# zhouyifan233/light-transport

Measured on AMD Instinct MI355X. Metric: photon_steps_per_sec, higher is better.
Workload: dtype f64

## Files before the change

### light_transport_amd/csrc/lt_api.cpp

```cpp
#include <hip/hip_runtime_api.h>

#include <dlfcn.h>

#include <algorithm>
#include <cmath>
#include <cctype>
#include <cstdarg>
#include <cstdio>
#include <cstdlib>
#include <cstring>
#include <limits>
#include <mutex>
#include <new>
#include <string>
#include <vector>

#include "lt_internal.hpp"

using namespace ltk;

static const size_t kMeshLdsBudget = 64 * 1024;

namespace {

// ... 635 lines not shown
    static WalkGate gates[16];
    return gates[device & 15];
}

hipError_t lane_event(LogLane& ln, hipStream_t s)
{
    if (ln.ev_used == ln.evs.size()) {
        hipEvent_t ev;
        hipError_t e = hipEventCreate(&ev);
        if (e != hipSuccess) return e;
        ln.evs.push_back(ev);
    }
    return hipEventRecord(ln.evs[ln.ev_used++], s);
}

int run_log_plan(LogRun& R, const LogPlan& plan, uint64_t offset, int* n_batches)
{
    lt_ctx* c = R.c;
    const LogGeom& G = R.G;
    const bool hot = G.bits2 != 0 && c->dmap_valid;
    const uint32_t n_hist = G.bits2 ? G.nb1 : G.n_tiles;
    LaunchCfg cfg = R.cfg;
    cfg.lds_bytes = walk_lds_bytes(R.v, R.P.n_media, R.P.n_layers, R.P.n_tris, R.P.n_nodes, n_hist);
    const int resident = walk_max_blocks_per_cu(R.v, cfg.threads, cfg.lds_bytes);
    if (resident <= 0) return c->fail(LT_E_HIP, "lt_launch: log-mode kernel not resident");
    int per_cu = c->blocks_per_cu > 0 ? c->blocks_per_cu : (plan.lanes >= 2 ? (resident + 1) / 2 : resident);
    if (plan.lanes >= 2 && c->knob.overlap_walk_bpc >= 1 && c->knob.overlap_walk_bpc <= 8) per_cu = (int)c->knob.overlap_walk_bpc;
    const unsigned long long cap = (unsigned long long)per_cu * (unsigned long long)c->prop.multiProcessorCount;
    if (plan.lanes >= 2) {
        const size_t gb = c->n_vox() * c->grid_elem();
        HIP_TRY(c, hipEventRecord(c->ev_fork, c->stream));
        for (int l = 1; l < plan.lanes; l++) {
            if (!c->lanes[l].stream) HIP_TRY(c, hipStreamCreateWithFlags(&c->lanes[l].stream, hipStreamNonBlocking));
            HIP_TRY(c, hipStreamWaitEvent(c->lanes[l].stream, c->ev_fork, 0));
            HIP_TRY(c, hipMemsetAsync(c->d_gridx[l - 1].p, 0, gb, c->lanes[l].stream));
        }
    }
    for (const auto& bt : plan.batches) {
        LogLane& ln = c->lanes[bt.first];
        hipStream_t s = ln.stream;
        uint32_t* meta = (uint32_t*)ln.meta.p;
        WalkParams P = R.P;
        P.n_photons = bt.second; P.photon_offset = offset;
        if (bt.first >= 1) P.grid = c->d_gridx[bt.first - 1].p;
        P.head = (unsigned long long*)ln.head.p;
        P.log_idx = (uint32_t*)ln.log_idx.p; P.log_val = ln.log_val.p; P.log_fill = (uint32_t*)ln.log_fill.p;
        P.log_next = meta + LM_NEXT; P.log_overflow = meta + LM_OVERFLOW; P.log_cap_chunks = plan.cap_chunks[bt.first];
// ... 14 lines not shown
        L.items2 = (uint32_t*)ln.items2.p; L.items_c = (uint32_t*)ln.items_c.p; L.items_r = (uint32_t*)ln.items_r.p;
        L.itab = (uint32_t*)ln.itab.p;
        L.meta = meta; L.job = (unsigned long long*)c->d_job.p; L.cap_chunks = P.log_cap_chunks;
        L.n_tiles = G.n_tiles; L.bits2 = G.bits2;
        L.grid = bt.first >= 1 ? c->d_gridx[bt.first - 1].p : c->d_grid.p; L.n_vox = c->n_vox(); L.tally = c->tally;
        L.nx = (uint32_t)c->nx; L.ny = (uint32_t)c->ny; L.nz = (uint32_t)c->nz; L.ntx = G.ntx; L.nty = G.nty;
        L.flush_atomic = 0;
        if (hot) { L.dmap = (const uint16_t*)c->d_dmap.p; L.dmeta = (const uint32_t*)c->d_dmeta.p; }

        HIP_TRY(c, hipMemsetAsync(ln.head.p, 0, sizeof(unsigned long long), s));
        HIP_TRY(c, hipMemsetAsync(meta, 0, LM_WORDS * 4, s));
        HIP_TRY(c, hipMemsetAsync(ln.hist.p, 0, (size_t)G.n_tiles * (G.bits2 ? kLogGroups2 : kLogGroups) * 4, s));
        HIP_TRY(c, hipMemsetAsync(ln.log_fill.p, 0, (size_t)P.log_cap_chunks * 4, s));
        if (G.bits2) HIP_TRY(c, hipMemsetAsync(ln.hist1.p, 0, (size_t)(hot ? log_max_digits() : G.nb1) * kLogGroups * 4, s));
        const bool last_batch = &bt == &plan.batches.back();
        const uint64_t waves_launched = (uint64_t)cfg.blocks * (uint64_t)(cfg.threads / 64);
        const bool big_enough = c->knob.tail_split >= 2 || bt.second >= kTailSplitMinPerWave * waves_launched;
        const bool split = R.v.mesh <= 1 && !R.v.table && !R.v.capture && c->knob.tail_split != 0 && big_enough &&
                           ((plan.lanes == 1 && (c->blocks_per_cu == 0 || c->knob.serial_walks > 0) && (!R.v.f32 || c->knob.tail_split >= 2)) ||
                            (plan.lanes > 1 && last_batch));
        L.alone = (plan.lanes == 1 && c->blocks_per_cu == 0 && !split) ? 1 : 0;
        if (c->knob.part_alone == 0 || c->knob.part_alone == 1) L.alone = (int)c->knob.part_alone;
        L.lds_part = c->knob.part_lds > 0 ? (int)(c->knob.part_lds & 7) : 0;
        Variant vw = R.v;
        if (split) {
            const size_t cap = (size_t)cfg.blocks * (size_t)(cfg.threads / 64) * kDumpPoolLanes;
            P.dump_max = c->knob.tail_split > 1 ? (uint32_t)std::min<long>(c->knob.tail_split, (long)kDumpPoolLanes) : kDumpMaxLanes;
            HIP_TRY(c, ln.pool.ensure(cap * (R.v.f32 ? sizeof(SurvD<float>) : sizeof(SurvD<double>))));
            HIP_TRY(c, ln.pool_n.ensure(4));
            if (!ln.tail_stream) HIP_TRY(c, hipStreamCreateWithFlags(&ln.tail_stream, hipStreamNonBlocking));
            if (!ln.ev_bulk) HIP_TRY(c, hipEventCreateWithFlags(&ln.ev_bulk, hipEventDisableTiming));
            if (!ln.ev_tail) HIP_TRY(c, hipEventCreateWithFlags(&ln.ev_tail, hipEventDisableTiming));
            HIP_TRY(c, hipMemsetAsync(ln.pool_n.p, 0, 4, s));
            P.pool = ln.pool.p; P.pool_n = (uint32_t*)ln.pool_n.p; P.pool_cap = (uint32_t)cap;
            vw.phase = 1;
        }
        const bool train = c->knob.serial_walks > 0;
        if (train) {
            WalkGate& g = walk_gate(c->device);
            std::lock_guard<std::mutex> lk(g.mu);
            if (g.last) HIP_TRY(c, hipStreamWaitEvent(s, g.last, 0));
        }
        HIP_TRY(c, lane_event(ln, s));
        HIP_TRY(c, launch_walk(P, vw, cfg, s));
        HIP_TRY(c, lane_event(ln, s));
        if (split) {
            HIP_TRY(c, hipEventRecord(ln.ev_bulk, s));
// ... 297 lines not shown
              uint64_t table_steps, uint32_t flags)
{
    CHECK_CTX(c);
    if (c->media.empty()) return c->fail(LT_E_STATE, "lt_launch: lt_set_media first");
    if (!c->have_layers && !c->have_mesh) return c->fail(LT_E_STATE, "lt_launch: lt_set_layers or lt_set_mesh first");
    if (!c->have_grid) return c->fail(LT_E_STATE, "lt_launch: lt_set_grid first");
    if (!c->have_source) return c->fail(LT_E_STATE, "lt_launch: lt_set_source first");
    const int n_media = (int)c->media.size();
    if (c->have_layers) {
        for (int32_t m : c->layer_medium) if (m >= n_media) return c->fail(LT_E_INVALID, "lt_launch: layer medium index %d >= %d media", m, n_media);
    } else {
        for (size_t i = 0; i < c->med_front.size(); i++)
            if (c->med_front[i] >= n_media || c->med_back[i] >= n_media || c->med_front[i] < -1 || c->med_back[i] < -1)
                return c->fail(LT_E_INVALID, "lt_launch: triangle %zu medium index out of range", i);
        if (c->start_medium < 0 || c->start_medium >= n_media) return c->fail(LT_E_INVALID, "lt_launch: start_medium out of range");
    }
    Variant v;
    v.f32 = (flags & LT_FLAG_F32_WALK) ? 1 : 0;
    v.mesh = c->have_mesh ? 1 : 0;
    v.table = rng_table ? 1 : 0;
    v.tally = c->tally;
    v.capture = c->max_vertices > 0 ? 1 : 0;
    v.phase = 0;
    if (v.capture && (v.f32 || v.table)) return c->fail(LT_E_UNSUPPORTED, "lt_launch: vertex capture runs the f64 walk with the XORWOW generator");
    if (c->on(c->knob.diag_no_tally)) v.tally = 3;
    if (v.table && v.f32) return c->fail(LT_E_UNSUPPORTED, "lt_launch: table RNG runs the f64 walk only");
    if (v.table && v.tally == LT_TALLY_F32) return c->fail(LT_E_UNSUPPORTED, "lt_launch: table RNG needs an f64 or u64fx tally");
    if (v.table && table_steps == 0) return c->fail(LT_E_INVALID, "lt_launch: table_steps == 0");
    BIND(c);
    int rc = upload_tables(c);
    if (rc) return rc;
    if (n_photons == 0) { c->timed = false; return LT_OK; }

    if (v.table) {
        const size_t bytes = (size_t)n_photons * (size_t)table_steps * 4 * sizeof(double);
        HIP_TRY(c, c->d_table.ensure(bytes));
        HIP_TRY(c, hipMemcpyAsync(c->d_table.p, rng_table, bytes, hipMemcpyHostToDevice, c->stream));
        HIP_TRY(c, hipStreamSynchronize(c->stream));
    }

    WalkParams P;
    std::memset(&P, 0, sizeof P);
    P.head = (unsigned long long*)c->d_head.p;
    P.n_photons = n_photons; P.photon_offset = photon_offset; P.seed = seed;
    const int pi = v.f32 ? 1 : 0;
    P.media = c->d_media[pi].p; P.zb = c->d_zb[pi].p; P.ifaces = c->d_if[pi].p; P.layer_medium = (const int32_t*)c->d_lm.p;
// ... 612 lines not shown
```

### light_transport_amd/csrc/lt_internal.hpp

```cpp
#pragma once
#include <hip/hip_runtime_api.h>
#include <stdint.h>

#include "../../include/lt.h"

namespace ltk {

template <typename R>
struct MedD {
    R mu_t, inv_mu_t, absorb, g;
    R n, one_m_g2, one_p_g2, inv_2g;
    R dep;
    R one_m_g, two_g;
    R pad_;
};

template <typename R>
struct IfD {
    R n_up, n_dn;
    R nr_down, nr_up;
};

template <typename R>
struct TriD {
// ... 85 lines not shown
    double corg[3], cinv[3];
    MarchGrid mg;
    void* pool;
    uint32_t* pool_n;
    uint32_t pool_cap;
    uint32_t dump_max;
    lt_vertex* vertices;
    uint32_t* vertex_counts;
    unsigned max_vertices;
};

struct LaunchCfg {
    int blocks, threads;
    size_t lds_bytes;
};

struct Variant {
    int f32;
    int mesh;
    int table;
    int tally;
    int capture;
    int phase;
};

hipError_t launch_walk(const WalkParams& P, const Variant& v, const LaunchCfg& cfg, hipStream_t s);
size_t walk_lds_bytes(const Variant& v, int n_media, int n_layers, int n_tris, int n_nodes, unsigned n_hist = 0);
int walk_max_blocks_per_cu(const Variant& v, int threads, size_t lds_bytes);

struct RenderParams {
    const void* tris;
    const void* nodes;
    const lt_surface_material* mats;
    const lt_point_light* lights;
    const int16_t* links;
    int n_tris, n_nodes, n_lights;
    int W, H, S, D;
    double cam[3], f_distance;
    const double* xs;
    const double* ys;
    double* rand_0;
    const double* rand_1;
    const int32_t* light_choice;
    double* image;
    int variant;
    int choices;
// ... 72 lines not shown
```

### light_transport_amd/csrc/lt_kernels.hip

```cpp
#include <hip/hip_runtime.h>

#define ROCRAND_DETAIL_BM_NOT_IN_STATE
#include <rocrand/rocrand_xorwow.h>
#include <rocrand/rocrand_uniform.h>

#include "lt_internal.hpp"

static_assert(sizeof(rocrand_state_xorwow) == 6 * sizeof(uint32_t), "rocrand_state_xorwow is not {d, x[5]}: SurvD::rng and the tail-split hand-over assume it");

namespace ltk {

#define LT_DEV __device__ __forceinline__
#define LT_PV(name, k) (sizeof(R) == 8 ? (R)P.name[k] : (R)P.f32.name[k])
#define LT_GV(name, k) (sizeof(R) == 8 ? (R)G.name[k] : (R)G.name##32[k])

#ifdef LT_K_IN_SGPR
LT_DEV double fma_k(double a, double b, double k) { double r; asm("v_fma_f64 %0, %1, %2, %3" : "=v"(r) : "v"(a), "v"(b), "s"(k)); return r; }
LT_DEV double fma_mk(double a, double k, double c) { return __builtin_fma(a, k, c); }
LT_DEV double mul_k(double a, double k) { return a * k; }
LT_DEV double fma_kk(double x, double k) { double r; asm("v_fma_f64 %0, %1, %2, %2" : "=v"(r) : "v"(x), "s"(k)); return r; }
#else
template <unsigned long long BITS> LT_DEV double fma_kb(double a, double b)
{
    double r;
// ... 731 lines not shown
        if (qn > 0 && (full || qn >= 64u || !__any(marching))) march_drain(tris, G, W, qn);
    }
    if (want) march_result(tris, nodes, n_nodes, (const int16_t*)nullptr, W, outside || heavy, px, py, pz, ux, uy, uz, tmax, prim, t_out);
    else { prim = -1; t_out = Mx<R>::inf(); }
}

template <typename R> LT_DEV R hg_pdf(R cos_t, R g)
{
    R denom = (R)1 + g * g + (R)2 * g * cos_t;
    return (R)0.07957747154594767 * ((R)1 - g * g) / (denom * Mx<R>::sqrt(denom));
}

template <typename R> LT_DEV R hg_sample(R xi, R g, R one_m_g2, R one_p_g2, R inv_2g)
{
    R c;
    if (g == 0) c = (R)2 * xi - (R)1;
    else {
        R t = Mx<R>::quot(one_m_g2, (R)1 - g + (R)2 * g * xi);
        c = (one_p_g2 - t * t) * inv_2g;
    }
    return Mx<R>::clamp_unit(c);
}

template <typename R> LT_DEV R hg_sample_walk(R xi, const MedD<R>* M)
{
    if (M->g == 0) return (R)2 * xi - (R)1;
    const R t = Mx<R>::quot(M->one_m_g2, M->two_g * xi + M->one_m_g);
    return (M->one_p_g2 - t * t) * M->inv_2g;
}

template <typename R> LT_DEV void onb(const R* n, R* v2, R* v3)
{
    if (Mx<R>::abs(n[0]) > Mx<R>::abs(n[1])) {
        R l = Mx<R>::sqrt(n[0] * n[0] + n[2] * n[2]);
        v2[0] = -n[2] / l; v2[1] = 0; v2[2] = n[0] / l;
    } else {
        R l = Mx<R>::sqrt(n[1] * n[1] + n[2] * n[2]);
        v2[0] = 0; v2[1] = n[2] / l; v2[2] = -n[1] / l;
    }
    cross3(n, v2, v3);
}

template <typename R, bool LEAN = false> LT_DEV void disk(R u0, R u1, R* d)
{
    R ox = (R)2 * u0 - (R)1, oy = (R)2 * u1 - (R)1;
    if (ox == 0 && oy == 0) { d[0] = 0; d[1] = 0; return; }
    R r, theta;
    if (Mx<R>::abs(ox) > Mx<R>::abs(oy)) { r = ox; theta = (R)0.7853981633974483 * (oy / ox); }
// ... 172 lines not shown
};

LT_DEV void lds_copy(void* dst, const void* src, size_t bytes)
{
    uint32_t* d = reinterpret_cast<uint32_t*>(dst);
    const uint32_t* s = reinterpret_cast<const uint32_t*>(src);
    for (size_t i = threadIdx.x; i < bytes / 4; i += blockDim.x) d[i] = s[i];
}

LT_DEV unsigned long long readlane64(unsigned long long v, int lane)
{
    unsigned lo = __builtin_amdgcn_readlane((unsigned)v, lane);
    unsigned hi = __builtin_amdgcn_readlane((unsigned)(v >> 32), lane);
    return ((unsigned long long)hi << 32) | lo;
}

template <typename T> LT_DEV T wave_sum(T v)
{
#pragma unroll
    for (int off = 32; off > 0; off >>= 1) v += __shfl_down(v, off, 64);
    return v;
}

template <typename R>
LT_DEV void record_vertex(const WalkParams& P, unsigned long long rel, unsigned& nv, R px, R py, R pz, R ux, R uy,
                          R uz, R w, int kind, int medium, unsigned step, R gx, R gy, R gz, R pdf_pos, R pdf_dir)
{
    if (nv < P.max_vertices) {
        lt_vertex* v = P.vertices + rel * (unsigned long long)P.max_vertices + nv;
        v->point[0] = (double)px; v->point[1] = (double)py; v->point[2] = (double)pz;
        v->direction[0] = (double)ux; v->direction[1] = (double)uy; v->direction[2] = (double)uz;
        v->g_norm[0] = (double)gx; v->g_norm[1] = (double)gy; v->g_norm[2] = (double)gz;
        v->throughput = (double)w; v->pdf_pos = (double)pdf_pos; v->pdf_dir = (double)pdf_dir;
        v->kind = kind; v->medium = medium; v->step = step; v->pad_ = 0;
        nv++;
        P.vertex_counts[rel] = nv;
    }
}

constexpr unsigned kLogExhausted = 0xfffffffeu;
template <int TALLY>
LT_DEV void emit_deposit(const WalkParams& P, bool has, unsigned idx, typename TallyT<TALLY>::type val,
                         unsigned& lg_cur, unsigned& lg_end, unsigned& lg_chunk, uint32_t* s_hist)
{
    typedef typename TallyT<TALLY>::type TV;
    if (P.log_idx == nullptr) {
        if (has) tally_add<TALLY>(P.grid, idx, val);
        return;
    }
    const unsigned long long m = __ballot(has);
    if (m == 0ull) return;
    const unsigned cnt = (unsigned)__popcll(m);
    if (lg_chunk != kLogExhausted && lg_end - lg_cur < cnt) {
        const int lane = threadIdx.x & 63;
        const unsigned grp = blockIdx.x & (kLogGroups - 1);
        if (lg_chunk < kLogExhausted && lane == 0) P.log_fill[lg_chunk] = lg_cur - lg_chunk * kLogChunk;
        unsigned c = 0;
        if (lane == 0) c = __hip_atomic_fetch_add(P.log_next + grp, 1u, __ATOMIC_RELAXED, __HIP_MEMORY_SCOPE_AGENT);
        c = grp + kLogGroups * __builtin_amdgcn_readfirstlane(c);
        if (c < P.log_cap_chunks) { lg_chunk = c; lg_cur = c * kLogChunk; lg_end = lg_cur + kLogChunk; }
        else { lg_chunk = kLogExhausted; lg_cur = lg_end = 0; }
    }
    if (lg_chunk == kLogExhausted) {
        if ((threadIdx.x & 63) == 0) __hip_atomic_fetch_add(P.log_overflow, cnt, __ATOMIC_RELAXED, __HIP_MEMORY_SCOPE_AGENT);
        if (has) {
            unsigned ntx = P.log_ntx, nty = P.log_nty;
            asm volatile("" : "+s"(ntx), "+s"(nty));
            const unsigned tile = idx >> kTileShift, tx = tile % ntx, ty = (tile / ntx) % nty,
                           tz = tile / (ntx * nty);
            const unsigned vx = (tx << kTileBX) | (idx & 31u), vy = (ty << kTileBY) | ((idx >> 5) & 31u),
                           vz = (tz << kTileBZ) | ((idx >> 10) & 15u);
            tally_add<TALLY>(P.grid, (vz * (unsigned)P.ny + vy) * (unsigned)P.nx + vx, val);
        }
        return;
    }
    if (has) {
        const unsigned rank = __builtin_amdgcn_mbcnt_hi((unsigned)(m >> 32), __builtin_amdgcn_mbcnt_lo((unsigned)m, 0u));
        P.log_idx[lg_cur + rank] = idx;
        reinterpret_cast<TV*>(P.log_val)[lg_cur + rank] = val;
        atomicAdd(&s_hist[idx >> P.log_hist_shift], 1u);
    }
    lg_cur += cnt;
}

constexpr unsigned kPacket = 64;
#ifndef LT_REFILL_MIN
#define LT_REFILL_MIN 4
#endif
constexpr unsigned kRefillMin = LT_REFILL_MIN;
#ifndef LT_QUERY_MIN
#define LT_QUERY_MIN 8
#endif
constexpr unsigned kQueryMin = LT_QUERY_MIN;
constexpr unsigned kQueryMinGlobal = 48;
#ifndef LT_QUERY_MAX_AGE
#define LT_QUERY_MAX_AGE 8
#endif
// ... 28 lines not shown
#define LT_WALK_NAME walk_kernel
#define LT_WALK_BATCH 0
#include "lt_walk_kernel.inc"
#undef LT_WALK_NAME
#undef LT_WALK_BATCH
#undef LT_INV_MODE
#define LT_INV_MODE LT_INV_MODE_MESH
#define LT_WALK_NAME walk_kernel_q
#define LT_WALK_BATCH 1
#include "lt_walk_kernel.inc"
#undef LT_WALK_NAME
#undef LT_WALK_BATCH
#undef LT_INV_MODE
#define LT_INV_MODE LT_INV_MODE_MARCH
#define LT_WALK_NAME walk_kernel_m
#define LT_WALK_BATCH 2
#include "lt_walk_kernel.inc"
#undef LT_WALK_NAME
#undef LT_WALK_BATCH
#undef LT_INV_MODE

typedef void (*WalkFn)(const WalkParams);

template <typename R, int GEOM, bool TABLE, bool CAPTURE>
static WalkFn pick_tally(int tally)
{
    switch (tally) {
    case LT_TALLY_F32:
        if constexpr (TABLE) return nullptr;
        else if constexpr (GEOM == 0) return walk_kernel<R, GEOM, TABLE, LT_TALLY_F32, CAPTURE>;
        else return walk_kernel_q<R, GEOM, TABLE, LT_TALLY_F32, CAPTURE>;
    case LT_TALLY_F64:
        if constexpr (GEOM == 0) return walk_kernel<R, GEOM, TABLE, LT_TALLY_F64, CAPTURE>;
        else return walk_kernel_q<R, GEOM, TABLE, LT_TALLY_F64, CAPTURE>;
    case LT_TALLY_U64FX:
        if constexpr (GEOM == 0) return walk_kernel<R, GEOM, TABLE, LT_TALLY_U64FX, CAPTURE>;
        else return walk_kernel_q<R, GEOM, TABLE, LT_TALLY_U64FX, CAPTURE>;
    case LT_TALLY_NONE:
        if constexpr (!TABLE && GEOM == 0 && !CAPTURE) return walk_kernel<R, GEOM, TABLE, LT_TALLY_NONE, false>; else return nullptr;
    }
    return nullptr;
}

template <typename R, bool CAPTURE>
static WalkFn pick_march(int tally)
{
    switch (tally) {
    case LT_TALLY_F32: return walk_kernel_m<R, 2, false, LT_TALLY_F32, CAPTURE>;
    case LT_TALLY_F64: return walk_kernel_m<R, 2, false, LT_TALLY_F64, CAPTURE>;
    case LT_TALLY_U64FX: return walk_kernel_m<R, 2, false, LT_TALLY_U64FX, CAPTURE>;
    }
    return nullptr;
}

template <typename R, bool TABLE, bool CAPTURE>
static WalkFn pick_geom(const Variant& v)
{
    if (v.mesh == 3) { if constexpr (!TABLE) return pick_march<R, CAPTURE>(v.tally); else return nullptr; }
    if (v.mesh == 0) return pick_tally<R, 0, TABLE, CAPTURE>(v.tally);
    if (v.mesh == 1) return pick_tally<R, 1, TABLE, CAPTURE>(v.tally);
    if constexpr (!TABLE) return pick_tally<R, 2, TABLE, CAPTURE>(v.tally); else return nullptr;
}

template <typename R, int PHASE>
static WalkFn pick_phase(int tally)
{
    switch (tally) {
    case LT_TALLY_F32: return walk_kernel<R, 0, false, LT_TALLY_F32, false, PHASE>;
    case LT_TALLY_F64: return walk_kernel<R, 0, false, LT_TALLY_F64, false, PHASE>;
    case LT_TALLY_U64FX: return walk_kernel<R, 0, false, LT_TALLY_U64FX, false, PHASE>;
    }
    return nullptr;
}

template <typename R, int PHASE>
static WalkFn pick_phase_q(int tally)
{
    switch (tally) {
    case LT_TALLY_F32: return walk_kernel_q<R, 1, false, LT_TALLY_F32, false, PHASE>;
    case LT_TALLY_F64: return walk_kernel_q<R, 1, false, LT_TALLY_F64, false, PHASE>;
    case LT_TALLY_U64FX: return walk_kernel_q<R, 1, false, LT_TALLY_U64FX, false, PHASE>;
    }
    return nullptr;
}

static WalkFn pick(const Variant& v)
{
    if (v.phase) {
        if (v.mesh > 1 || v.table || v.capture) return nullptr;
        if (v.mesh == 1) {
            if (v.phase == 1) return v.f32 ? pick_phase_q<float, 1>(v.tally) : pick_phase_q<double, 1>(v.tally);
            return v.f32 ? pick_phase_q<float, 2>(v.tally) : pick_phase_q<double, 2>(v.tally);
        }
        if (v.phase == 1) return v.f32 ? pick_phase<float, 1>(v.tally) : pick_phase<double, 1>(v.tally);
        return v.f32 ? pick_phase<float, 2>(v.tally) : pick_phase<double, 2>(v.tally);
    }
    if (v.capture) return (v.f32 || v.table) ? nullptr : pick_geom<double, false, true>(v);
    if (v.f32) return v.table ? nullptr : pick_geom<float, false, false>(v);
    return v.table ? pick_geom<double, true, false>(v) : pick_geom<double, false, false>(v);
}

size_t walk_lds_bytes(const Variant& v, int n_media, int n_layers, int n_tris, int n_nodes, unsigned n_hist)
{
    if (v.mesh) n_layers = 0;
    if (v.mesh != 1) { n_tris = 0; n_nodes = 0; }
    return v.f32 ? LdsLayout<float>(n_media, n_layers, n_tris, n_nodes, n_hist, v.mesh == 3 ? 4 * sizeof(MarchWave<float>) : 0).total
                 : LdsLayout<double>(n_media, n_layers, n_tris, n_nodes, n_hist, v.mesh == 3 ? 4 * sizeof(MarchWave<double>) : 0).total;
}

int walk_max_blocks_per_cu(const Variant& v, int threads, size_t lds_bytes)
{
    WalkFn fn = pick(v);
    if (!fn) return 0;
    int nb = 0;
    if (hipOccupancyMaxActiveBlocksPerMultiprocessor(&nb, reinterpret_cast<const void*>(fn), threads, lds_bytes) != hipSuccess)
        return 0;
    return nb;
}

hipError_t launch_walk(const WalkParams& Pin, const Variant& v, const LaunchCfg& cfg, hipStream_t s)
{
    WalkFn fn = pick(v);
    if (!fn) return hipErrorInvalidValue;
    WalkParams P = Pin;
    if (v.mesh) P.n_layers = 0; else { P.n_tris = 0; P.n_nodes = 0; }
    if (cfg.lds_bytes > 64 * 1024) {
        hipError_t e = hipFuncSetAttribute(reinterpret_cast<const void*>(fn),
                                           hipFuncAttributeMaxDynamicSharedMemorySize, (int)cfg.lds_bytes);
        if (e != hipSuccess) return e;
    }
    hipLaunchKernelGGL(fn, dim3(cfg.blocks), dim3(cfg.threads), cfg.lds_bytes, s, P);
    return hipGetLastError();
}

__global__ void k_intersect_rays(const TriD<double>* tris, const NodeD<double>* nodes, int n_tris, int n_nodes,
                                 const double* o, const double* d, const double* tmax, size_t n, int use_bvh,
                                 const MarchGrid G, const int16_t* links, int32_t* prim, double* t)
{
    size_t i = (size_t)blockIdx.x * blockDim.x + threadIdx.x;
    if (use_bvh == 2) {
        __shared__ MarchWave<double> mw[4];
        const bool want = i < n;
        const size_t k = want ? i : 0;
        int pi; double tt;
        march_service<double>(tris, nodes, n_nodes, G, &mw[threadIdx.x >> 6], want, o[3 * k], o[3 * k + 1], o[3 * k + 2], d[3 * k], d[3 * k + 1],
                              d[3 * k + 2], tmax ? tmax[k] : __builtin_huge_val(), 0.0, pi, tt);
// ... 698 lines not shown
```

### light_transport_amd/csrc/lt_walk_kernel.inc

```
#ifndef LT_MED
#define LT_MED(i) reinterpret_cast<const MedD<R>*>(reinterpret_cast<const unsigned char*>(s_med) + __umul24((unsigned)(i), (unsigned)sizeof(MedD<R>)))
#endif
#if LT_WALK_BATCH != 2
template <typename R, int GEOM, bool TABLE, int TALLY, bool CAPTURE, int PHASE = 0>
#else
template <typename R, int GEOM, bool TABLE, int TALLY, bool CAPTURE>
#endif
#if LT_WALK_BATCH == 0 && defined(LT_SLAB_VGPR_CAP)
__attribute__((amdgpu_num_vgpr(LT_SLAB_VGPR_CAP)))
#endif
__global__ void __launch_bounds__(256, (sizeof(R) == 8 ? (GEOM == 0 ? LT_F64_SLAB_WAVES : (GEOM == 2 ? LT_F64_GLOBAL_WAVES : LT_F64_WAVES)) : (GEOM == 0 ? LT_F32_WAVES : 4))) LT_WALK_NAME(const WalkParams P)
{
    constexpr bool MESH = GEOM != 0;
#if LT_WALK_BATCH == 2
    constexpr int PHASE = 0;
#endif
#if LT_WALK_PRIO
    __builtin_amdgcn_s_setprio(LT_WALK_PRIO);
#endif
    extern __shared__ __attribute__((aligned(16))) unsigned char lds_raw[];
    const LdsLayout<R> L(P.n_media, P.n_layers, GEOM == 1 ? P.n_tris : 0, GEOM == 1 ? P.n_nodes : 0,
                         P.log_idx ? P.log_n_hist : 0u, LT_WALK_BATCH == 2 ? 4 * sizeof(MarchWave<R>) : 0);
    uint32_t* s_hist = reinterpret_cast<uint32_t*>(lds_raw + L.off_hist);
    if (P.log_idx) for (unsigned t = threadIdx.x; t < P.log_n_hist; t += blockDim.x) s_hist[t] = 0;
    double* s_cnt = reinterpret_cast<double*>(lds_raw + L.off_cnt);
    const MedD<R>* s_med = reinterpret_cast<const MedD<R>*>(lds_raw + L.off_media);
    const R* s_zb = reinterpret_cast<const R*>(lds_raw + L.off_zb);
    const int32_t* s_lm = reinterpret_cast<const int32_t*>(lds_raw + L.off_lm);
    const IfD<R>* s_if = reinterpret_cast<const IfD<R>*>(lds_raw + L.off_if);
    const TriD<R>* s_tris = GEOM == 2 ? reinterpret_cast<const TriD<R>*>(P.tris)
                                      : reinterpret_cast<const TriD<R>*>(lds_raw + L.off_tris);
    const NodeD<R>* s_nodes = GEOM == 2 ? reinterpret_cast<const NodeD<R>*>(P.nodes)
                                        : reinterpret_cast<const NodeD<R>*>(lds_raw + L.off_nodes);

    const int16_t* s_links = !MESH || !P.links ? nullptr
                             : (GEOM == 1 ? reinterpret_cast<const int16_t*>(lds_raw + L.off_links) : P.links);
    if (threadIdx.x < 8) s_cnt[threadIdx.x] = 0.0;
    R* s_frame = reinterpret_cast<R*>(lds_raw + L.off_frame);
// ... 203 lines not shown
                    P.vertex_counts[id] = 0;
                    if (alive) {
                        R pdf_pos = 1;
                        if (P.src_type == LT_SRC_COSINE_QUAD) {
                            const R e1[3] = {(R)P.src_e1[0], (R)P.src_e1[1], (R)P.src_e1[2]}, e2[3] = {(R)P.src_e2[0], (R)P.src_e2[1], (R)P.src_e2[2]};
                            R cr[3]; cross3(e1, e2, cr);
                            pdf_pos = (R)1 / Mx<R>::sqrt(dot3(cr, cr));
                        }
                        record_vertex<R>(P, id, nv, px, py, pz, ux, uy, uz, w, LT_VERTEX_LIGHT, cur, 0u, (R)P.src_dir[0], (R)P.src_dir[1],
                                         (R)P.src_dir[2], pdf_pos, e_pdf_dir);
                    }
                }
                if constexpr (TABLE) {
                    unsigned long long cap = P.table_steps > grp ? P.table_steps - grp : 0ull;
                    if (cap < (unsigned long long)max_steps) max_steps = (unsigned)cap;
                }
            }
        }
        if constexpr (PHASE == 1) {
            if (q_done && pk_next >= pk_end && !dumped) {
                const unsigned long long am = __ballot(alive);
                const unsigned na = (unsigned)__popcll(am);
                if (na != 0u && na <= P.dump_max) {
                    emit_deposit<TALLY>(P, pend_idx != kNoVoxel, pend_idx, pend_val, lg_cur, lg_end, lg_chunk, s_hist);
                    pend_idx = kNoVoxel;
                    const int leader = __ffsll((long long)am) - 1;
                    unsigned base = 0;
                    if (lane == leader) base = __hip_atomic_fetch_add(P.pool_n, na, __ATOMIC_RELAXED, __HIP_MEMORY_SCOPE_AGENT);
                    base = (unsigned)__builtin_amdgcn_readlane((int)base, leader);
                    if (alive) {
                        const unsigned slot = base + __builtin_amdgcn_mbcnt_hi((unsigned)(am >> 32), __builtin_amdgcn_mbcnt_lo((unsigned)am, 0u));
                        if (slot < P.pool_cap) {
                            SurvD<R>& S = reinterpret_cast<SurvD<R>*>(P.pool)[slot];
                            S.p[0] = px; S.p[1] = py; S.p[2] = pz; S.u[0] = ux; S.u[1] = uy; S.u[2] = uz; S.w = w; S.sleft = sleft;
                            S.pid = 0ull; S.cur = cur; S.step = step;
                            __builtin_memcpy(S.rng, &rng, sizeof S.rng);
#if LT_WALK_BATCH == 1
                            if constexpr (!TABLE) {
                                S.q_pend = q_pend ? 1u : 0u;
                                S.held[0] = __builtin_bit_cast(uint32_t, q_u1); S.held[1] = __builtin_bit_cast(uint32_t, q_u2);
                                S.held[2] = __builtin_bit_cast(uint32_t, q_u3);
                                q_pend = false;
                            }
#else
                            S.q_pend = 0u;
#endif
                            alive = false;
// ... 214 lines not shown
#endif
            }
        }
#if defined(LT_DIAG_MESH)
        {
            const unsigned long long gm = __ballot(go), bm = __ballot(go && hit_tri >= 0);
            dg_go += __popcll(gm);
            if (bm) { dg_bnd_it++; dg_bnd += __popcll(bm); }
            if (gm & ~bm) { dg_int_it++; dg_int += __popcll(gm & ~bm); }
        }
#endif
#if defined(LT_DIAG_MESH)
        const long long dg_t1 = clock64();
#endif
        if (go) {
            {
                const MedD<R>* Mp = LT_MED(MESH ? cur : s_lm[cur]);
                const R mu_t = Mp->mu_t;
#else
        unsigned f_idx = kNoVoxel;
        TV f_val = 0;
        if (alive) {
            if (step >= max_steps) {
                atomicAdd(&s_cnt[CW_CAPPED], (double)w); alive = false;
            } else {
                step++;
                acc_steps++;
                float clr = -1.0f;
                if constexpr (GEOM == 2) {
                    if (P.mg.cell) clr = march_clearance<R>(P.mg, px, py, pz);
                } else if constexpr (MESH) {
                    if (P.clear) {
                        const R cx = (px - LT_PV(corg, 0)) * LT_PV(cinv, 0), cy = (py - LT_PV(corg, 1)) * LT_PV(cinv, 1),
                                cz = (pz - LT_PV(corg, 2)) * LT_PV(cinv, 2);
                        if (cx >= 0 && cx < LT_PV(cdim, 0) && cy >= 0 && cy < LT_PV(cdim, 1) && cz >= 0 && cz < LT_PV(cdim, 2))
                            clr = __uint_as_float(P.clear[((size_t)(int)cz * P.cny + (int)cy) * P.cnx + (int)cx].x);
                    }
                }
                R u1;
                typename HeldU<R, TABLE>::type x0, x2, x3;
                if constexpr (TABLE) {
                    const double* t = P.table + ((pid - P.photon_offset) * P.table_steps + grp) * 4;
                    x0 = (R)(1.0 - t[0]); u1 = (R)(1.0 - t[1]); x2 = (R)(1.0 - t[2]); x3 = (R)(1.0 - t[3]);
                } else {
                    x0 = HeldU<R, TABLE>::draw(&rng);
                    u1 = Mx<R>::uniform32(&rng);
                    x2 = HeldU<R, TABLE>::draw(&rng);
                    x3 = HeldU<R, TABLE>::draw(&rng);
                }
                grp++;
                const MedD<R>* Mp = LT_MED(MESH ? cur : s_lm[cur]);
                const R mu_t = Mp->mu_t;
                if (sleft == 0) sleft = HeldU<R, TABLE>::neg_log(x0, s_math);
                const R s = (mu_t > 0) ? sleft * Mp->inv_mu_t : inf;

                R tb = inf; int hit_tri = -1;
                if constexpr (!MESH) {
                    if (uz != 0) {
                        const R dz = (uz > 0 ? s_zb[cur + 1] : s_zb[cur]) - pz;
                        const R guard = sizeof(R) == 8 ? (R)(1.0 + 1e-12) : (R)(1.0 + 1e-5);
                        const bool near = !(Mx<R>::abs(dz) > s * Mx<R>::abs(uz) * guard);
                        if (__any(near)) {
                            R den = uz;
                            asm volatile("" : "+v"(den));
                            if (near) tb = dz / den;
                        }
                    }
                } else {
                    const bool query = !(s < (R)clr);
                    if (query) {
                        R o[3] = {px, py, pz}, d[3] = {ux, uy, uz}, th;
                        nearest_bvh_walk(s_tris, s_nodes, P.n_nodes, s_links, o, d, s, hit_tri, th);
                        if (hit_tri >= 0) tb = th;
                    }
                }
#endif
                const bool at_boundary = MESH ? (hit_tri >= 0) : (tb <= s);
                if (!at_boundary && !(s < inf)) {
                    atomicAdd(&s_cnt[MESH ? CW_ESC_MESH : CW_CAPPED], (double)w); alive = false;
                } else if (at_boundary) {
                    px += ux * tb; py += uy * tb; pz += uz * tb;
                    sleft -= tb * mu_t;
                    if (!(sleft > 0)) sleft = 0;
                    if constexpr (!MESH) {
                        const bool down = uz > 0;
                        const int k = down ? cur + 1 : cur, next = down ? cur + 1 : cur - 1;
                        pz = s_zb[k];
                        const IfD<R> F = s_if[k];
                        const R Nr = down ? F.nr_down : F.nr_up;
                        R ct;
                        const R Rf = boundary_planar(uz, down ? F.n_up : F.n_dn, down ? F.n_dn : F.n_up, Nr, &ct);
                        const bool refl = HeldU<R, TABLE>::get(x3) <= Rf;
                        const bool gone = !refl && (next < 0 || next >= P.n_layers);
                        if constexpr (CAPTURE) if (P.vertices)
                            record_vertex<R>(P, pid - P.photon_offset, nv, px, py, pz, ux, uy, uz, w,
                                             refl ? LT_VERTEX_REFLECTIVE : LT_VERTEX_TRANSMISSIVE, cur, step, (R)0, (R)0, down ? (R)-1 : (R)1, (R)0,
                                             gone ? (R)0 : (refl ? Rf : (R)1 - Rf));
                        if (refl) uz = -uz;
                        else if (gone) { atomicAdd(&s_cnt[next < 0 ? CW_ESC_TOP : CW_ESC_BOT], (double)w); alive = false; }
                        else { ux *= Nr; uy *= Nr; uz = down ? ct : -ct; cur = next; }
                    } else {
                    R nf[3], n1 = Mp->n, n2; int next;
                    {
                        const TriD<R>* T = &s_tris[hit_tri];
                        R tn[3] = {T->n[0], T->n[1], T->n[2]};
                        R d[3] = {ux, uy, uz};
                        R dn = dot3(d, tn);
                        R sg = dn > 0 ? (R)-1 : (R)1;
                        nf[0] = sg * tn[0]; nf[1] = sg * tn[1]; nf[2] = sg * tn[2];
                        next = dn > 0 ? T->med_front : T->med_back;
                        n2 = next >= 0 ? s_med[next].n : n1;
                    }
                    R d[3] = {ux, uy, uz}, ct, refr[3];
                    R Rf = boundary(d, nf, n1, n2, &ct, refr);
                    if constexpr (CAPTURE) if (P.vertices) {
                        const bool refl = HeldU<R, TABLE>::get(x3) <= Rf;
                        const bool leaves = !refl && next < 0;
                        record_vertex<R>(P, pid - P.photon_offset, nv, px, py, pz, ux, uy, uz, w,
                                         refl ? LT_VERTEX_REFLECTIVE : LT_VERTEX_TRANSMISSIVE, cur, step, nf[0], nf[1], nf[2], (R)0,
                                         leaves ? (R)0 : (refl ? Rf : (R)1 - Rf));
                    }
                    if (HeldU<R, TABLE>::get(x3) <= Rf) {
// ... 3 lines not shown
                    } else if (next < 0) {
                        atomicAdd(&s_cnt[CW_ESC_MESH], (double)w); alive = false;
                    } else {
                        ux = refr[0]; uy = refr[1]; uz = refr[2];
                        px -= eps * nf[0]; py -= eps * nf[1]; pz -= eps * nf[2];
                        cur = next;
                    }
                    }
                } else {
                    px += ux * s; py += uy * s; pz += uz * s;
                    sleft = 0;
                    const R dw = w * Mp->absorb;
                    if constexpr (CAPTURE) if (P.vertices) {
                        const R ct_c = hg_sample_walk(u1, Mp);
                        record_vertex<R>(P, pid - P.photon_offset, nv, px, py, pz, ux, uy, uz, w, LT_VERTEX_VOLUME, cur, step, (R)0, (R)0, (R)0,
                                         (R)0, (w - dw > 0) ? hg_pdf(-ct_c, Mp->g) : (R)0);
                    }
                    const R fx = (px - gx0) * ivx, fy = (py - gy0) * ivy, fz = (pz - gz0) * ivz;
                    const unsigned vx = (unsigned)(int)fx, vy = (unsigned)(int)fy, vz = (unsigned)(int)fz;
                    bool inside;
                    if constexpr (!MESH) inside = (int)(Mx<R>::sign_word(fx) | Mx<R>::sign_word(fy) | Mx<R>::sign_word(fz)) >= 0 &&
                                                  vx < (unsigned)P.nx && vy < (unsigned)P.ny && vz < (unsigned)P.nz;
                    else inside = fx >= 0 && fx < fnx && fy >= 0 && fy < fny && fz >= 0 && fz < fnz;
                    const unsigned idx = P.log_idx
                        ? (((__umul24(__umul24(vz >> kTileBZ, P.log_nty) + (vy >> kTileBY), P.log_ntx) + (vx >> kTileBX)) << kTileShift)
                           | ((vz & 15u) << 10) | ((vy & 31u) << 5) | (vx & 31u))
                        : (vz * (unsigned)P.ny + vy) * (unsigned)P.nx + vx;
                    const TV q = tally_quantum<TALLY, R>(w * Mp->dep);
                    const bool same = inside && idx == pend_idx;
                    const bool flush = inside && !same;
                    f_idx = flush ? pend_idx : kNoVoxel; f_val = pend_val;
                    pend_val = same ? pend_val + q : (flush ? q : pend_val);
                    pend_idx = flush ? idx : pend_idx;
                    acc_abs += inside ? (double)dw : 0.0;
                    acc_lost += inside ? 0.0 : (double)dw;
                    w -= dw;
                    if (!(w > 0)) alive = false;
                    else {
                        R u[3] = {ux, uy, uz};
                        spin<R, TABLE>(u, hg_sample_walk(u1, Mp), x2, s_math);
                        ux = u[0]; uy = u[1]; uz = u[2];
                        if (w < (R)1e-4) {
                            if (HeldU<R, TABLE>::get(x3) <= (R)0.1) { atomicAdd(&s_cnt[CW_ROULETTE], -9.0 * (double)w); w *= (R)10; }
                            else { atomicAdd(&s_cnt[CW_ROULETTE], (double)w); alive = false; }
                        }
                    }
                }
            }
        }
#if LT_WALK_BATCH && defined(LT_DIAG_MESH)
        dg_clk_bnd += clock64() - dg_t1;
#endif
        emit_deposit<TALLY>(P, f_idx != kNoVoxel, f_idx, f_val, lg_cur, lg_end, lg_chunk, s_hist);
    }
    emit_deposit<TALLY>(P, pend_idx != kNoVoxel, pend_idx, pend_val, lg_cur, lg_end, lg_chunk, s_hist);
    if (P.log_idx && lg_chunk < kLogExhausted && (threadIdx.x & 63) == 0) P.log_fill[lg_chunk] = lg_cur - lg_chunk * kLogChunk;

#if LT_WALK_BATCH && defined(LT_DIAG_MESH)
#if LT_WALK_BATCH == 2
    if (blockIdx.x == 7 && threadIdx.x == 0) {
        const double tot = (double)(clock64() - dg_clk_all);
        printf("[march diag] iterations %llu, cycles per iteration %.0f | alive %.1f, preparing %.1f | share of the wave's time: prepare %.3f, march round %.3f "
               "(in %.3f of iterations, %.1f lanes), drain %.3f (in %.3f of iterations, %.1f items), resolve %.3f, complete %.3f | complete %.1f lanes: "
               "boundary in %.3f of iterations (%.1f lanes), interaction in %.3f (%.1f lanes) | refills %.3f of iterations (%.1f lanes)\n",
               dg_iter, tot / dg_iter, (double)dg_alive / dg_iter, (double)dg_prep / dg_iter, dgm_clk[0] / tot, dgm_clk[1] / tot, (double)dg_trav_it / dg_iter,
               dg_trav_it ? (double)dg_trav / dg_trav_it : 0.0, dgm_clk[2] / tot, (double)dg_bvh_it / dg_iter, dg_bvh_it ? (double)dg_bvh / dg_bvh_it : 0.0,
               dgm_clk[3] / tot, dg_clk_bnd / tot, (double)dg_go / dg_iter, (double)dg_bnd_it / dg_iter, dg_bnd_it ? (double)dg_bnd / dg_bnd_it : 0.0,
               (double)dg_int_it / dg_iter, dg_int_it ? (double)dg_int / dg_int_it : 0.0, (double)dg_refill_it / dg_iter, dg_refill_it ? (double)dg_refill / dg_refill_it : 0.0);
    }
#else
    if (blockIdx.x == 7 && threadIdx.x == 0) {
        const double tot = (double)(clock64() - dg_clk_all);
        printf("[mesh diag] cycles per service %.0f; share of the wave's time: services %.3f, complete-stage %.3f; cycles per iteration %.0f\n",
               dg_trav_it ? (double)dg_clk_srv / dg_trav_it : 0.0, dg_clk_srv / tot, dg_clk_bnd / tot, tot / dg_iter);
    }
#endif
    if (blockIdx.x == 7 && threadIdx.x == 0)
        printf("[mesh diag] iterations %llu | alive %.1f/64 | prepare %.1f | waiting for a query %.1f | traversals: %.3f of iterations, %.1f lanes each | "
// ... 39 lines not shown
```

Before: 89.49 billion.

## Specialize f64 slab walk kernel by tally route and straighten branchy hot paths

Adds a compile-time ROUTE parameter so the f64 slab walk kernel is instantiated separately for direct-grid tallies and log-mode tallies. This removes the runtime log_idx checks from the hot deposit and indexing code. It also makes the HG sampling, the boundary test and the spin path branchless for f64, computing both sides and selecting. Opaque asm barriers keep the compiler from reintroducing branches. The cost is extra kernel instantiations and some speculative arithmetic on lanes that would otherwise have skipped it.

Measured after the change: 73.99 billion. 17.3% lower.

```diff
diff --git a/light_transport_amd/csrc/lt_api.cpp b/light_transport_amd/csrc/lt_api.cpp
--- a/light_transport_amd/csrc/lt_api.cpp
+++ b/light_transport_amd/csrc/lt_api.cpp
@@ -681,7 +681,8 @@
     const uint32_t n_hist = G.bits2 ? G.nb1 : G.n_tiles;
     LaunchCfg cfg = R.cfg;
     cfg.lds_bytes = walk_lds_bytes(R.v, R.P.n_media, R.P.n_layers, R.P.n_tris, R.P.n_nodes, n_hist);
-    const int resident = walk_max_blocks_per_cu(R.v, cfg.threads, cfg.lds_bytes);
+    Variant vlog = R.v; vlog.log = 1;
+    const int resident = walk_max_blocks_per_cu(vlog, cfg.threads, cfg.lds_bytes);
     if (resident <= 0) return c->fail(LT_E_HIP, "lt_launch: log-mode kernel not resident");
     int per_cu = c->blocks_per_cu > 0 ? c->blocks_per_cu : (plan.lanes >= 2 ? (resident + 1) / 2 : resident);
     if (plan.lanes >= 2 && c->knob.overlap_walk_bpc >= 1 && c->knob.overlap_walk_bpc <= 8) per_cu = (int)c->knob.overlap_walk_bpc;
@@ -742,7 +743,7 @@
         L.alone = (plan.lanes == 1 && c->blocks_per_cu == 0 && !split) ? 1 : 0;
         if (c->knob.part_alone == 0 || c->knob.part_alone == 1) L.alone = (int)c->knob.part_alone;
         L.lds_part = c->knob.part_lds > 0 ? (int)(c->knob.part_lds & 7) : 0;
-        Variant vw = R.v;
+        Variant vw = vlog;
         if (split) {
             const size_t cap = (size_t)cfg.blocks * (size_t)(cfg.threads / 64) * kDumpPoolLanes;
             P.dump_max = c->knob.tail_split > 1 ? (uint32_t)std::min<long>(c->knob.tail_split, (long)kDumpPoolLanes) : kDumpMaxLanes;
@@ -1086,6 +1087,7 @@
     v.tally = c->tally;
     v.capture = c->max_vertices > 0 ? 1 : 0;
     v.phase = 0;
+    v.log = 0;
     if (v.capture && (v.f32 || v.table)) return c->fail(LT_E_UNSUPPORTED, "lt_launch: vertex capture runs the f64 walk with the XORWOW generator");
     if (c->on(c->knob.diag_no_tally)) v.tally = 3;
     if (v.table && v.f32) return c->fail(LT_E_UNSUPPORTED, "lt_launch: table RNG runs the f64 walk only");
diff --git a/light_transport_amd/csrc/lt_internal.hpp b/light_transport_amd/csrc/lt_internal.hpp
--- a/light_transport_amd/csrc/lt_internal.hpp
+++ b/light_transport_amd/csrc/lt_internal.hpp
@@ -131,6 +131,7 @@
     int tally;
     int capture;
     int phase;
+    int log;
 };
 
 hipError_t launch_walk(const WalkParams& P, const Variant& v, const LaunchCfg& cfg, hipStream_t s);
diff --git a/light_transport_amd/csrc/lt_kernels.hip b/light_transport_amd/csrc/lt_kernels.hip
--- a/light_transport_amd/csrc/lt_kernels.hip
+++ b/light_transport_amd/csrc/lt_kernels.hip
@@ -777,8 +777,15 @@
     return Mx<R>::clamp_unit(c);
 }
 
-template <typename R> LT_DEV R hg_sample_walk(R xi, const MedD<R>* M)
-{
+template <typename R, bool STRAIGHT = false> LT_DEV R hg_sample_walk(R xi, const MedD<R>* M)
+{
+    if constexpr (STRAIGHT) {
+        const R iso = (R)2 * xi - (R)1;
+        const R t = Mx<R>::quot(M->one_m_g2, M->two_g * xi + M->one_m_g);
+        R c = (M->one_p_g2 - t * t) * M->inv_2g;
+        asm volatile("" : "+v"(c));
+        return M->g == 0 ? iso : c;
+    }
     if (M->g == 0) return (R)2 * xi - (R)1;
     const R t = Mx<R>::quot(M->one_m_g2, M->two_g * xi + M->one_m_g);
     return (M->one_p_g2 - t * t) * M->inv_2g;
@@ -997,6 +1004,15 @@
     return v;
 }
 
+template <bool DIRECT> LT_DEV void cnt_add(double* s_cnt, int which, double v)
+{
+    if constexpr (DIRECT) {
+        unsigned k = (unsigned)which;
+        asm volatile("" : "+v"(k));
+        atomicAdd(s_cnt + k, v);
+    } else atomicAdd(&s_cnt[which], v);
+}
+
 template <typename R>
 LT_DEV void record_vertex(const WalkParams& P, unsigned long long rel, unsigned& nv, R px, R py, R pz, R ux, R uy,
                           R uz, R w, int kind, int medium, unsigned step, R gx, R gy, R gz, R pdf_pos, R pdf_dir)
@@ -1014,40 +1030,48 @@
 }
 
 constexpr unsigned kLogExhausted = 0xfffffffeu;
-template <int TALLY>
+template <int TALLY, int ROUTE = 0>
 LT_DEV void emit_deposit(const WalkParams& P, bool has, unsigned idx, typename TallyT<TALLY>::type val,
                          unsigned& lg_cur, unsigned& lg_end, unsigned& lg_chunk, uint32_t* s_hist)
 {
     typedef typename TallyT<TALLY>::type TV;
-    if (P.log_idx == nullptr) {
+    if (ROUTE == 1 || (ROUTE == 0 && P.log_idx == nullptr)) {
         if (has) tally_add<TALLY>(P.grid, idx, val);
         return;
     }
     const unsigned long long m = __ballot(has);
-    if (m == 0ull) return;
     const unsigned cnt = (unsigned)__popcll(m);
-    if (lg_chunk != kLogExhausted && lg_end - lg_cur < cnt) {
-        const int lane = threadIdx.x & 63;
-        const unsigned grp = blockIdx.x & (kLogGroups - 1);
-        if (lg_chunk < kLogExhausted && lane == 0) P.log_fill[lg_chunk] = lg_cur - lg_chunk * kLogChunk;
-        unsigned c = 0;
-        if (lane == 0) c = __hip_atomic_fetch_add(P.log_next + grp, 1u, __ATOMIC_RELAXED, __HIP_MEMORY_SCOPE_AGENT);
-        c = grp + kLogGroups * __builtin_amdgcn_readfirstlane(c);
-        if (c < P.log_cap_chunks) { lg_chunk = c; lg_cur = c * kLogChunk; lg_end = lg_cur + kLogChunk; }
-        else { lg_chunk = kLogExhausted; lg_cur = lg_end = 0; }
-    }
-    if (lg_chunk == kLogExhausted) {
-        if ((threadIdx.x & 63) == 0) __hip_atomic_fetch_add(P.log_overflow, cnt, __ATOMIC_RELAXED, __HIP_MEMORY_SCOPE_AGENT);
-        if (has) {
-            unsigned ntx = P.log_ntx, nty = P.log_nty;
-            asm volatile("" : "+s"(ntx), "+s"(nty));
-            const unsigned tile = idx >> kTileShift, tx = tile % ntx, ty = (tile / ntx) % nty,
-                           tz = tile / (ntx * nty);
-            const unsigned vx = (tx << kTileBX) | (idx & 31u), vy = (ty << kTileBY) | ((idx >> 5) & 31u),
-                           vz = (tz << kTileBZ) | ((idx >> 10) & 15u);
-            tally_add<TALLY>(P.grid, (vz * (unsigned)P.ny + vy) * (unsigned)P.nx + vx, val);
-        }
-        return;
+    bool rare = true;
+    if constexpr (ROUTE == 2) {
+        rare = !(cnt - 1u < lg_end - lg_cur);
+        if (rare && cnt == 0u) return;
+    } else {
+        if (m == 0ull) return;
+    }
+    if (rare) {
+        if (lg_chunk != kLogExhausted && lg_end - lg_cur < cnt) {
+            const int lane = threadIdx.x & 63;
+            const unsigned grp = blockIdx.x & (kLogGroups - 1);
+            if (lg_chunk < kLogExhausted && lane == 0) P.log_fill[lg_chunk] = lg_cur - lg_chunk * kLogChunk;
+            unsigned c = 0;
+            if (lane == 0) c = __hip_atomic_fetch_add(P.log_next + grp, 1u, __ATOMIC_RELAXED, __HIP_MEMORY_SCOPE_AGENT);
+            c = grp + kLogGroups * __builtin_amdgcn_readfirstlane(c);
+            if (c < P.log_cap_chunks) { lg_chunk = c; lg_cur = c * kLogChunk; lg_end = lg_cur + kLogChunk; }
+            else { lg_chunk = kLogExhausted; lg_cur = lg_end = 0; }
+        }
+        if (lg_chunk == kLogExhausted) {
+            if ((threadIdx.x & 63) == 0) __hip_atomic_fetch_add(P.log_overflow, cnt, __ATOMIC_RELAXED, __HIP_MEMORY_SCOPE_AGENT);
+            if (has) {
+                unsigned ntx = P.log_ntx, nty = P.log_nty;
+                asm volatile("" : "+s"(ntx), "+s"(nty));
+                const unsigned tile = idx >> kTileShift, tx = tile % ntx, ty = (tile / ntx) % nty,
+                               tz = tile / (ntx * nty);
+                const unsigned vx = (tx << kTileBX) | (idx & 31u), vy = (ty << kTileBY) | ((idx >> 5) & 31u),
+                               vz = (tz << kTileBZ) | ((idx >> 10) & 15u);
+                tally_add<TALLY>(P.grid, (vz * (unsigned)P.ny + vy) * (unsigned)P.nx + vx, val);
+            }
+            return;
+        }
     }
     if (has) {
         const unsigned rank = __builtin_amdgcn_mbcnt_hi((unsigned)(m >> 32), __builtin_amdgcn_mbcnt_lo((unsigned)m, 0u));
@@ -1122,19 +1146,23 @@
 
 typedef void (*WalkFn)(const WalkParams);
 
+template <typename R, int GEOM, bool TABLE, bool CAPTURE> constexpr bool kRouted = sizeof(R) == 8 && GEOM == 0 && !TABLE && !CAPTURE;
+
 template <typename R, int GEOM, bool TABLE, bool CAPTURE>
 static WalkFn pick_tally(int tally)
 {
     switch (tally) {
     case LT_TALLY_F32:
-        if constexpr (TABLE) return nullptr;
+        if constexpr (TABLE || kRouted<R, GEOM, TABLE, CAPTURE>) return nullptr;
         else if constexpr (GEOM == 0) return walk_kernel<R, GEOM, TABLE, LT_TALLY_F32, CAPTURE>;
         else return walk_kernel_q<R, GEOM, TABLE, LT_TALLY_F32, CAPTURE>;
     case LT_TALLY_F64:
-        if constexpr (GEOM == 0) return walk_kernel<R, GEOM, TABLE, LT_TALLY_F64, CAPTURE>;
+        if constexpr (kRouted<R, GEOM, TABLE, CAPTURE>) return nullptr;
+        else if constexpr (GEOM == 0) return walk_kernel<R, GEOM, TABLE, LT_TALLY_F64, CAPTURE>;
         else return walk_kernel_q<R, GEOM, TABLE, LT_TALLY_F64, CAPTURE>;
     case LT_TALLY_U64FX:
-        if constexpr (GEOM == 0) return walk_kernel<R, GEOM, TABLE, LT_TALLY_U64FX, CAPTURE>;
+        if constexpr (kRouted<R, GEOM, TABLE, CAPTURE>) return nullptr;
+        else if constexpr (GEOM == 0) return walk_kernel<R, GEOM, TABLE, LT_TALLY_U64FX, CAPTURE>;
         else return walk_kernel_q<R, GEOM, TABLE, LT_TALLY_U64FX, CAPTURE>;
     case LT_TALLY_NONE:
         if constexpr (!TABLE && GEOM == 0 && !CAPTURE) return walk_kernel<R, GEOM, TABLE, LT_TALLY_NONE, false>; else return nullptr;
@@ -1165,10 +1193,22 @@
 template <typename R, int PHASE>
 static WalkFn pick_phase(int tally)
 {
-    switch (tally) {
+    if constexpr (sizeof(R) == 8 && PHASE == 1) return nullptr;
+    else switch (tally) {
     case LT_TALLY_F32: return walk_kernel<R, 0, false, LT_TALLY_F32, false, PHASE>;
     case LT_TALLY_F64: return walk_kernel<R, 0, false, LT_TALLY_F64, false, PHASE>;
     case LT_TALLY_U64FX: return walk_kernel<R, 0, false, LT_TALLY_U64FX, false, PHASE>;
+    }
+    return nullptr;
+}
+
+template <int PHASE, int ROUTE>
+static WalkFn pick_route(int tally)
+{
+    switch (tally) {
+    case LT_TALLY_F32: return walk_kernel<double, 0, false, LT_TALLY_F32, false, PHASE, ROUTE>;
+    case LT_TALLY_F64: return walk_kernel<double, 0, false, LT_TALLY_F64, false, PHASE, ROUTE>;
+    case LT_TALLY_U64FX: return walk_kernel<double, 0, false, LT_TALLY_U64FX, false, PHASE, ROUTE>;
     }
     return nullptr;
 }
@@ -1186,6 +1226,10 @@
 
 static WalkFn pick(const Variant& v)
 {
+    if (!v.f32 && v.mesh == 0 && !v.table && !v.capture && v.phase != 2 && v.tally != LT_TALLY_NONE) {
+        if (v.phase == 1) return v.log ? pick_route<1, 2>(v.tally) : nullptr;
+        return v.log ? pick_route<0, 2>(v.tally) : pick_route<0, 1>(v.tally);
+    }
     if (v.phase) {
         if (v.mesh > 1 || v.table || v.capture) return nullptr;
         if (v.mesh == 1) {
@@ -1222,6 +1266,7 @@
 {
     WalkFn fn = pick(v);
     if (!fn) return hipErrorInvalidValue;
+    if ((v.log != 0) != (Pin.log_idx != nullptr)) return hipErrorInvalidValue;
     WalkParams P = Pin;
     if (v.mesh) P.n_layers = 0; else { P.n_tris = 0; P.n_nodes = 0; }
     if (cfg.lds_bytes > 64 * 1024) {
diff --git a/light_transport_amd/csrc/lt_walk_kernel.inc b/light_transport_amd/csrc/lt_walk_kernel.inc
--- a/light_transport_amd/csrc/lt_walk_kernel.inc
+++ b/light_transport_amd/csrc/lt_walk_kernel.inc
@@ -1,7 +1,9 @@
 #ifndef LT_MED
 #define LT_MED(i) reinterpret_cast<const MedD<R>*>(reinterpret_cast<const unsigned char*>(s_med) + __umul24((unsigned)(i), (unsigned)sizeof(MedD<R>)))
 #endif
-#if LT_WALK_BATCH != 2
+#if LT_WALK_BATCH == 0
+template <typename R, int GEOM, bool TABLE, int TALLY, bool CAPTURE, int PHASE = 0, int ROUTE = 0>
+#elif LT_WALK_BATCH == 1
 template <typename R, int GEOM, bool TABLE, int TALLY, bool CAPTURE, int PHASE = 0>
 #else
 template <typename R, int GEOM, bool TABLE, int TALLY, bool CAPTURE>
@@ -12,8 +14,12 @@
 __global__ void __launch_bounds__(256, (sizeof(R) == 8 ? (GEOM == 0 ? LT_F64_SLAB_WAVES : (GEOM == 2 ? LT_F64_GLOBAL_WAVES : LT_F64_WAVES)) : (GEOM == 0 ? LT_F32_WAVES : 4))) LT_WALK_NAME(const WalkParams P)
 {
     constexpr bool MESH = GEOM != 0;
+    constexpr bool kStraight = !MESH && sizeof(R) == 8;
 #if LT_WALK_BATCH == 2
     constexpr int PHASE = 0;
+#endif
+#if LT_WALK_BATCH != 0
+    constexpr int ROUTE = 0;
 #endif
 #if LT_WALK_PRIO
     __builtin_amdgcn_s_setprio(LT_WALK_PRIO);
@@ -263,7 +269,7 @@
                 const unsigned long long am = __ballot(alive);
                 const unsigned na = (unsigned)__popcll(am);
                 if (na != 0u && na <= P.dump_max) {
-                    emit_deposit<TALLY>(P, pend_idx != kNoVoxel, pend_idx, pend_val, lg_cur, lg_end, lg_chunk, s_hist);
+                    emit_deposit<TALLY, ROUTE>(P, pend_idx != kNoVoxel, pend_idx, pend_val, lg_cur, lg_end, lg_chunk, s_hist);
                     pend_idx = kNoVoxel;
                     const int leader = __ffsll((long long)am) - 1;
                     unsigned base = 0;
@@ -524,7 +530,7 @@
         TV f_val = 0;
         if (alive) {
             if (step >= max_steps) {
-                atomicAdd(&s_cnt[CW_CAPPED], (double)w); alive = false;
+                cnt_add<kStraight>(s_cnt, CW_CAPPED, (double)w); alive = false;
             } else {
                 step++;
                 acc_steps++;
@@ -554,19 +560,19 @@
                 const MedD<R>* Mp = LT_MED(MESH ? cur : s_lm[cur]);
                 const R mu_t = Mp->mu_t;
                 if (sleft == 0) sleft = HeldU<R, TABLE>::neg_log(x0, s_math);
-                const R s = (mu_t > 0) ? sleft * Mp->inv_mu_t : inf;
+                R s_any = sleft * Mp->inv_mu_t;
+                if constexpr (kStraight) asm volatile("" : "+v"(s_any));
+                const R s = (mu_t > 0) ? s_any : inf;
 
                 R tb = inf; int hit_tri = -1;
                 if constexpr (!MESH) {
-                    if (uz != 0) {
-                        const R dz = (uz > 0 ? s_zb[cur + 1] : s_zb[cur]) - pz;
-                        const R guard = sizeof(R) == 8 ? (R)(1.0 + 1e-12) : (R)(1.0 + 1e-5);
-                        const bool near = !(Mx<R>::abs(dz) > s * Mx<R>::abs(uz) * guard);
-                        if (__any(near)) {
-                            R den = uz;
-                            asm volatile("" : "+v"(den));
-                            if (near) tb = dz / den;
-                        }
+                    const R dz = (uz > 0 ? s_zb[cur + 1] : s_zb[cur]) - pz;
+                    const R guard = sizeof(R) == 8 ? (R)(1.0 + 1e-12) : (R)(1.0 + 1e-5);
+                    const bool near = uz != 0 && !(Mx<R>::abs(dz) > s * Mx<R>::abs(uz) * guard);
+                    if (__any(near)) {
+                        R den = uz;
+                        asm volatile("" : "+v"(den));
+                        if (near) tb = dz / den;
                     }
                 } else {
                     const bool query = !(s < (R)clr);
@@ -579,7 +585,7 @@
 #endif
                 const bool at_boundary = MESH ? (hit_tri >= 0) : (tb <= s);
                 if (!at_boundary && !(s < inf)) {
-                    atomicAdd(&s_cnt[MESH ? CW_ESC_MESH : CW_CAPPED], (double)w); alive = false;
+                    cnt_add<kStraight>(s_cnt, MESH ? CW_ESC_MESH : CW_CAPPED, (double)w); alive = false;
                 } else if (at_boundary) {
                     px += ux * tb; py += uy * tb; pz += uz * tb;
                     sleft -= tb * mu_t;
@@ -599,7 +605,7 @@
                                              refl ? LT_VERTEX_REFLECTIVE : LT_VERTEX_TRANSMISSIVE, cur, step, (R)0, (R)0, down ? (R)-1 : (R)1, (R)0,
                                              gone ? (R)0 : (refl ? Rf : (R)1 - Rf));
                         if (refl) uz = -uz;
-                        else if (gone) { atomicAdd(&s_cnt[next < 0 ? CW_ESC_TOP : CW_ESC_BOT], (double)w); alive = false; }
+                        else if (gone) { cnt_add<kStraight>(s_cnt, next < 0 ? CW_ESC_TOP : CW_ESC_BOT, (double)w); alive = false; }
                         else { ux *= Nr; uy *= Nr; uz = down ? ct : -ct; cur = next; }
                     } else {
                     R nf[3], n1 = Mp->n, n2; int next;
@@ -649,7 +655,8 @@
                     if constexpr (!MESH) inside = (int)(Mx<R>::sign_word(fx) | Mx<R>::sign_word(fy) | Mx<R>::sign_word(fz)) >= 0 &&
                                                   vx < (unsigned)P.nx && vy < (unsigned)P.ny && vz < (unsigned)P.nz;
                     else inside = fx >= 0 && fx < fnx && fy >= 0 && fy < fny && fz >= 0 && fz < fnz;
-                    const unsigned idx = P.log_idx
+                    const bool tiled = ROUTE == 2 || (ROUTE == 0 && P.log_idx != nullptr);
+                    const unsigned idx = tiled
                         ? (((__umul24(__umul24(vz >> kTileBZ, P.log_nty) + (vy >> kTileBY), P.log_ntx) + (vx >> kTileBX)) << kTileShift)
                            | ((vz & 15u) << 10) | ((vy & 31u) << 5) | (vx & 31u))
                         : (vz * (unsigned)P.ny + vy) * (unsigned)P.nx + vx;
@@ -662,14 +669,15 @@
                     acc_abs += inside ? (double)dw : 0.0;
                     acc_lost += inside ? 0.0 : (double)dw;
                     w -= dw;
-                    if (!(w > 0)) alive = false;
-                    else {
+                    const bool more = w > 0;
+                    if (!more) alive = false;
+                    if ((kStraight && PHASE != 2) || more) {
                         R u[3] = {ux, uy, uz};
-                        spin<R, TABLE>(u, hg_sample_walk(u1, Mp), x2, s_math);
+                        spin<R, TABLE>(u, hg_sample_walk<R, kStraight>(u1, Mp), x2, s_math);
                         ux = u[0]; uy = u[1]; uz = u[2];
-                        if (w < (R)1e-4) {
-                            if (HeldU<R, TABLE>::get(x3) <= (R)0.1) { atomicAdd(&s_cnt[CW_ROULETTE], -9.0 * (double)w); w *= (R)10; }
-                            else { atomicAdd(&s_cnt[CW_ROULETTE], (double)w); alive = false; }
+                        if (more && w < (R)1e-4) {
+                            if (HeldU<R, TABLE>::get(x3) <= (R)0.1) { cnt_add<kStraight>(s_cnt, CW_ROULETTE, -9.0 * (double)w); w *= (R)10; }
+                            else { cnt_add<kStraight>(s_cnt, CW_ROULETTE, (double)w); alive = false; }
                         }
                     }
                 }
@@ -678,9 +686,9 @@
 #if LT_WALK_BATCH && defined(LT_DIAG_MESH)
         dg_clk_bnd += clock64() - dg_t1;
 #endif
-        emit_deposit<TALLY>(P, f_idx != kNoVoxel, f_idx, f_val, lg_cur, lg_end, lg_chunk, s_hist);
+        emit_deposit<TALLY, ROUTE>(P, f_idx != kNoVoxel, f_idx, f_val, lg_cur, lg_end, lg_chunk, s_hist);
     }
-    emit_deposit<TALLY>(P, pend_idx != kNoVoxel, pend_idx, pend_val, lg_cur, lg_end, lg_chunk, s_hist);
+    emit_deposit<TALLY, ROUTE>(P, pend_idx != kNoVoxel, pend_idx, pend_val, lg_cur, lg_end, lg_chunk, s_hist);
     if (P.log_idx && lg_chunk < kLogExhausted && (threadIdx.x & 63) == 0) P.log_fill[lg_chunk] = lg_cur - lg_chunk * kLogChunk;
 
 #if LT_WALK_BATCH && defined(LT_DIAG_MESH)
```
